# Gaius-Augustus/Augustus

Hardware: AMD Instinct MI355X
Metric: Mbp DNA decoded/sec (whole node), ab-initio human model (higher is better)
Workload: dtype f64; 1 GPU; synthetic uniform-random DNA, 100 contigs x 1000000 bp per GPU, --species=human ab initio (47 states, sample=0); pieces_in_flight_per_gpu=100, batches_in_flight_per_gpu=1

## Files before the change

augustus_amd/csrc/device/decoder.hip:

```cpp
#include <hip/hip_runtime.h>
#include <sys/mman.h>
#include <algorithm>
#include <map>
#include <array>
#include <cmath>
#include <unordered_map>
#include <cstdio>
#include <cstdlib>
#include <cstring>
#include <future>
#include <memory>
#include <mutex>
#include <set>
#include <string>
#include <system_error>
#include <thread>
#include <atomic>
#include <chrono>
#include <vector>
#include "kernels.h"
#include "dense.h"
#include "layout.h"
#include "launch.h"
#include "assmemo.h"
// ... 313 lines not shown

__global__ void __launch_bounds__(256) kTileCross(BatchView B) {
    const int64_t gt = (int64_t)blockIdx.x * 256 + threadIdx.x;
    if (gt < B.N / WAVE) tileCrossOne(B, gt);
}
__global__ void __launch_bounds__(64) kSegFinalize(BatchView B) {
    const int p = blockIdx.x * 64 + threadIdx.x;
    if (p < B.nPieces) segFinalizePiece(B, p);
}
__global__ void __launch_bounds__(64) kBacktrace(const DevTables *T, BatchView B) { backtracePiece(*T, B, blockIdx.x); }
struct GatherWin { int64_t o, gb0, poolOff, fxOff, fOff; int32_t b0, b1, g0, nSlots, nPl, r0, nRows, pad; };
__global__ void __launch_bounds__(256) kGatherWindows(BatchView V, const GatherWin *W, Item *outItems, uint64_t *outFx, const double *mat, double *outF, int S) {
    __shared__ uint32_t sc[256];
    __shared__ uint64_t running;
    const GatherWin w = W[blockIdx.x];
    const int t = threadIdx.x;
    if (t == 0) running = 0;
    __syncthreads();
    for (int base = w.b0; base <= w.b1; base += 256) {
        const int q = base + t;
        const uint32_t cnt = q <= w.b1 ? V.blkCnt[(w.gb0 + q) * 2 + 1] : 0;
        sc[t] = cnt;
        __syncthreads();
        for (int off = 1; off < 256; off <<= 1) {
            const uint32_t v = t >= off ? sc[t - off] : 0;
            __syncthreads();
            sc[t] += v;
            __syncthreads();
        }
        const uint64_t dst = (uint64_t)w.poolOff + running + (sc[t] - cnt);
        if (cnt) {
            const Item *src = V.items + V.blkOff[(w.gb0 + q) * 2 + 1];
            for (uint32_t i = 0; i < cnt; i++) outItems[dst + i] = src[i];
        }
        __syncthreads();
        if (t == 255) running += sc[255];
        __syncthreads();
    }
    const int64_t nFx = (int64_t)w.nPl * 2 * w.nSlots;
    for (int64_t i = t; i < nFx; i += 256) {
        const int pl = (int)(i / (2 * w.nSlots)), rev = (int)((i / w.nSlots) % 2), g = w.g0 + (int)(i % w.nSlots);
        outFx[w.fxOff + i] = V.fx[(int64_t)pl * V.N * NFX + fidx(w.o + g, rev ? FX_INR : FX_INF, NFX)];
    }
    if (mat && outF)
        for (int64_t i = t; i < (int64_t)w.nRows * S; i += 256) outF[w.fOff + i] = mat[(w.o + 1 + w.r0) * S + i];
}
__global__ void __launch_bounds__(256) kPatchItems(BatchView B, const uint64_t *idx, const double *te, int n) {
    const int i = blockIdx.x * blockDim.x + threadIdx.x;
    if (i < n) B.items[idx[i]].te = te[i];
}

namespace augx { namespace dev {
#define AUGX_BY_BLK(f, ...) do { if (blk == 8) f##8(__VA_ARGS__); else if (blk == 4) f##4(__VA_ARGS__); else f##2(__VA_ARGS__); } while (0)
void launchTrellis(int blk, int mode, bool ties, unsigned grid, hipStream_t st, const DevTables *T, const BatchView *B) { AUGX_BY_BLK(launchTrellis_, mode, ties, grid, st, T, B); }
void launchCand(int blk, bool multi, bool dense, unsigned grid, hipStream_t st, const DevTables *T, const BatchView &W) { AUGX_BY_BLK(launchCand_, multi, dense, grid, st, T, W); }
void launchForward(int blk, unsigned grid, hipStream_t st, const DevTables *T, const BatchView *B) { AUGX_BY_BLK(launchForward_, grid, st, T, B); }
void launchDense(int blk, int mode, bool ties, unsigned grid, hipStream_t st, const DevTables *T, const BatchView *B) { AUGX_BY_BLK(launchDense_, mode, ties, grid, st, T, B); }
void launchUtrDesc(int blk, unsigned grid, hipStream_t st, const DevTables *T, const BatchView &W) { AUGX_BY_BLK(launchUtrDesc_, grid, st, T, W); }
#undef AUGX_BY_BLK
}}

struct augx_decoder {
    const augx_model *model = nullptr;
    int device = 0;
    hipStream_t stream = nullptr;
    DevTables hostT;
    DevTables *dT = nullptr;
    std::vector<void *> tableBufs;
    bool debugCells = false;
    int blk = 8;
    int nCU = 256;
    int share = 1;
    std::multimap<size_t, void *> pool;
    std::unordered_map<void *, size_t> live;
    std::atomic<size_t> pooledBytes{0};
    std::mutex poolMu;
    std::vector<hipStream_t> copyStreams;
    bool dense = false;
    bool countNearTies = false;
    int64_t nearTies = 0, nearTiePieces = 0;
    double mallocSeconds = 0, mallocBytes = 0;
    bool exactMulti = true;
};

namespace {
int snippetCacheReplay(augx_decoder *d, augx_batch *b, int64_t &nPatched, bool fromLists, const double *mat);
int utrCachesReplay(augx_decoder *d, augx_batch *b, const double *mat, bool &rebuilt);
std::mutex g_regMu;
std::vector<augx_decoder *> g_decoders;
constexpr size_t POOL_CAP_BYTES = (size_t)250 << 30;
size_t sizeClass(size_t bytes) {
    if (bytes < ((size_t)1 << 20)) return (bytes + 4095) & ~(size_t)4095;
    size_t p2 = (size_t)1 << 20;
    while (p2 < bytes) p2 <<= 1;
    const size_t step = p2 >> 4;
    return (bytes + step - 1) / step * step;
}
void poolReleaseLocked(augx_decoder *d) {
    for (auto &kv : d->pool) (void)hipFree(kv.second);
    d->pool.clear();
    d->pooledBytes = 0;
}
void poolRelease(augx_decoder *d) {
    std::lock_guard<std::mutex> lk(d->poolMu);
    poolReleaseLocked(d);
}
hipError_t devMalloc(augx_decoder *d, void **out, size_t bytes) {
// ... 47 lines not shown
    d->pool.emplace(it->second, p);
    d->pooledBytes += it->second;
    d->live.erase(it);
}
struct DevBuf {
    augx_decoder *d = nullptr;
    void *p = nullptr;
    DevBuf() = default;
    DevBuf(DevBuf &&o) noexcept : d(o.d), p(o.p) { o.p = nullptr; }
    ~DevBuf() { reset(); }
    void reset() { devFree(d, p); p = nullptr; }
    explicit operator bool() const { return p != nullptr; }
    template <class T> T *as() const { return (T *)p; }
    int alloc(augx_decoder *dec, size_t bytes, const std::string &what) {
        reset();
        d = dec;
        const char *fail = getenv("AUGX_FAIL_ALLOC");
        const hipError_t e = fail && *fail && what.find(fail) != std::string::npos ? hipErrorOutOfMemory : devMalloc(d, &p, bytes);
        if (e == hipSuccess) return AUGX_OK;
        (void)hipGetLastError();
        p = nullptr;
        if (e == hipErrorOutOfMemory) { setLastError(what); return AUGX_E_NOMEM; }
        setLastError(std::string("HIP error: ") + hipGetErrorString(e) + " (" + what + ")");
        return AUGX_E_HIP;
    }
};
}


constexpr int NARR = 26;
struct augx_batch {
    augx_decoder *dec = nullptr;
    BatchLayout L;
    BatchView V;
    BatchView *dV = nullptr;
    std::vector<DevBuf> bufs;
    int32_t *blkMinMax = nullptr;
    int32_t *stairInfo = nullptr;
    int nPlAlloc = 0;
    int64_t listCapAlloc = 0;
    bool listsReady = false;
    int64_t *dListOffs = nullptr;
    DevBuf planeBufs[NARR];
    bool utrScanned = false;
    hipEvent_t ev[4] = {nullptr, nullptr, nullptr, nullptr};
    hipEvent_t evFwd = nullptr;
    uint64_t nItems = 0, nPairs = 0;
    DevBuf itemBuf;
    DevBuf udBuf;
    uint64_t nDescs = 0;
    bool decoded = false;
    bool itemsVerified = false;
    SegPlan plan;
    int chunkTotPlanes = 1;
    std::vector<int64_t> hListOffs;
    bool memoReplayed = false;
    DevBuf laSwBuf;
    size_t nLaSw = 0;
    std::vector<std::shared_ptr<augx::dev::AssMemoReplay>> memoOf;
};

namespace {

int ensureArrays(augx_batch *b, int nPl, int64_t listCap, bool *grown = nullptr) {
    if (nPl <= b->nPlAlloc && listCap <= b->listCapAlloc) return 0;
    if (grown) *grown = true;
    if (nPl < b->nPlAlloc) nPl = b->nPlAlloc;
    if (listCap < b->listCapAlloc) listCap = b->listCapAlloc;
    BatchView &V = b->V;
    const int64_t N = b->L.N, LC = listCap > 0 ? listCap : 1;
    struct Slot { void **field; size_t elem; int64_t count; int planes; };
    const Slot slots[NARR] = {
        {(void **)&V.fx, sizeof(uint64_t), N * NFX, nPl},          {(void **)&V.plsR, sizeof(double), N * 3, nPl},
        {(void **)&V.ldEnt, sizeof(IntronStart), LC, nPl},         {(void **)&V.rdEnt, sizeof(IntronStart), LC, nPl},
        {(void **)&V.laPls, sizeof(double), LC * 3, nPl},          {(void **)&V.laFx, sizeof(uint64_t), LC * 3, nPl},
        {(void **)&V.lrEt, sizeof(double), LC * 3, nPl},           {(void **)&V.lrFx, sizeof(uint64_t), LC * 3, nPl},
        {(void **)&V.atgD, sizeof(double), LC * 3, nPl},           {(void **)&V.atgFx, sizeof(uint64_t), LC, nPl},
        {(void **)&V.rsFx, sizeof(uint64_t), LC * 3, nPl},
        {(void **)&V.laPos, sizeof(int32_t), LC, 1},               {(void **)&V.laVal, sizeof(double), LC * 3, 1},
        {(void **)&V.lrPos, sizeof(int32_t), LC, 1},               {(void **)&V.lrVal, sizeof(double), LC * 3, 1},
        {(void **)&V.ldVal, sizeof(double), LC * 3, 1},            {(void **)&V.rdVal, sizeof(double), LC * 3, 1},
        {(void **)&V.atgPos, sizeof(int32_t), LC, 1},              {(void **)&V.rsPos, sizeof(int32_t), LC, 1},
        {(void **)&V.rsBegin, sizeof(double), LC, 1},
        {(void **)&V.tfSite, sizeof(USite), b->dec->dense ? LC : 1, 1}, {(void **)&V.laSite, sizeof(USite), b->dec->dense ? LC : 1, 1},
        {(void **)&V.fsSite, sizeof(USite), b->dec->dense ? LC : 1, 1}, {(void **)&V.lrSite, sizeof(USite), b->dec->dense ? LC : 1, 1},
        {(void **)&V.tmSite, sizeof(USite), b->dec->dense ? LC : 1, 1}, {(void **)&V.rtSite, sizeof(USite), b->dec->dense ? LC : 1, 1}};
    const std::string what = "augx: out of device memory for the candidate-list / per-GC-class arrays (" + std::to_string(nPl) + " classes in one piece); decode fewer bases per batch";
    for (int i = 0; i < NARR; i++) {
        const bool isN = i < 2;
        if (isN && nPl == b->nPlAlloc && b->planeBufs[i]) continue;
        if (const int rc = b->planeBufs[i].alloc(b->dec, (size_t)slots[i].planes * (size_t)slots[i].count * slots[i].elem, what)) {
            b->nPlAlloc = 0; b->listCapAlloc = 0;
            for (int k = 0; k < NARR; k++) { b->planeBufs[k].reset(); *slots[k].field = nullptr; }
            return rc;
        }
        *slots[i].field = b->planeBufs[i].p;
    }
    b->nPlAlloc = nPl;
    b->listCapAlloc = listCap;
    return 0;
}

}

extern "C" {

// ... 196 lines not shown
    if (!d->dense) {
        keep(V.bp, Z.N * SP);
        keep(V.bpChain, Z.N * 8);
    } else {
        keep(V.bpD, Z.N * d->hostT.S);
        keep(V.ufx, Z.N * NUFX); keep(V.ucnt, Z.N * NUCNT); keep(V.usig, Z.N * NUSIG);
    }
    if (d->debugCells || d->dense) keep(V.cells, Z.N * d->hostT.S);
    if (d->countNearTies) keep(V.nearTie, n);
    if (getenv("AUGX_PROF")) { keep(V.prof, (int64_t)n * 56 + 64); if (!rc && hipMemset(V.prof, 0, ((size_t)n * 56 + 64) * 8) != hipSuccess) { setLastError("augx_batch_create: hipMemset failed"); return AUGX_E_HIP; } }
    if (!d->dense) { keep(V.vig, Z.N); keep(V.longV, Z.N * 6); }
    keep(V.listCnt, n); keep(b->dListOffs, n + 1);
    V.listOffs = b->dListOffs;
    if (rc || (rc = ensureArrays(b.get(), 1, 0))) return rc;
    V.blk = d->blk;
    V.nBlk = Z.N / V.blk;
    keep(V.blkCnt, V.nBlk * 2); keep(V.blkSplit, V.nBlk * 3); keep(V.blkOff, V.nBlk * 2);
    keep(V.candAlloc, 1);
    if (d->dense && d->hostT.utr) { keep(V.udOff, V.nBlk); keep(V.udCnt, V.nBlk); }
    keep(V.lnv, n); keep(V.status, n); keep(V.finalState, n); keep(V.pathCount, n);
    {
        std::vector<double> v;
        {
            std::lock_guard<std::mutex> lk(g_tss0Mu);
            if (!g_tss0Of.empty() && d->dense && d->hostT.utr)
                for (int p = 0; p < n; p++) {
                    auto it = g_tss0Of.find(pieces[p].seq);
                    if (it == g_tss0Of.end()) continue;
                    if (v.empty()) v.assign((size_t)n * 2, std::nan(""));
                    v[(size_t)p * 2] = it->second[0]; v[(size_t)p * 2 + 1] = it->second[1];
                }
        }
        if (!v.empty()) {
            double *dv = nullptr;
            keep(dv, (int64_t)n * 2);
            if (rc) return rc;
            if (hipMemcpy(dv, v.data(), sizeof(double) * v.size(), hipMemcpyHostToDevice) != hipSuccess) { setLastError("augx_batch_create: upload failed"); return AUGX_E_HIP; }
            V.tss0 = dv;
        }
    }
    keep(V.pathRec, Z.pathCap * 3);
    b->plan = planSegments(L, d->model->m.t, d->nCU / d->share > 0 ? d->nCU / d->share : 1, d->dense ? -1 : 0);
    SegDesc *dSegs = nullptr; int32_t *dSeg0 = nullptr;
    const int nSegs = (int)b->plan.segs.size();
    keep(dSegs, nSegs); keep(dSeg0, n + 1);
    V.nSegs = nSegs; V.segs = dSegs; V.pieceSeg0 = dSeg0; V.segCheckTiles = b->plan.checkTiles;
    if (const char *e = getenv("AUGX_SEG_CHECK_TILES")) V.segCheckTiles = atoi(e);
    keep(V.segStop, nSegs); keep(V.segStatus, nSegs); keep(V.segD, nSegs); keep(V.brkPos, nSegs); keep(V.brkOff, nSegs);
    keep(V.segStop2, nSegs); keep(V.segD2, nSegs); keep(V.pieceCovered, n);
    if (b->plan.cut()) {
        keep(V.ckRing, (int64_t)nSegs * 2 * WAVE * SP); keep(V.ckCol, Z.N / WAVE * SP);
        keep(V.tileMinEop, Z.N / WAVE); keep(V.tileCross, Z.N / WAVE);
    }
    keep(b->dV, 1);
    if (rc) return rc;
    const double tAlloc = getenv("AUGX_TIMING") ? std::chrono::duration<double>(std::chrono::steady_clock::now().time_since_epoch()).count() : 0.0;
    HIP_TRY(hipMemcpy(dOff, L.off.data(), sizeof(int64_t) * (n + 1), hipMemcpyHostToDevice));
    HIP_TRY(hipMemcpy(dLen, L.len.data(), sizeof(int32_t) * n, hipMemcpyHostToDevice));
    HIP_TRY(hipMemcpy(dIk, L.initKind.data(), sizeof(int32_t) * n, hipMemcpyHostToDevice));
    HIP_TRY(hipMemcpy(dTk, L.termKind.data(), sizeof(int32_t) * n, hipMemcpyHostToDevice));
    HIP_TRY(hipMemcpy(dCp, L.chunkPiece.data(), sizeof(int32_t) * L.nChunks, hipMemcpyHostToDevice));
    HIP_TRY(hipMemcpy(dSegs, b->plan.segs.data(), sizeof(SegDesc) * nSegs, hipMemcpyHostToDevice));
    HIP_TRY(hipMemcpy(dSeg0, b->plan.pieceSeg0.data(), sizeof(int32_t) * (n + 1), hipMemcpyHostToDevice));
    HIP_TRY(hipMemset(dRaw, 'n', (size_t)Z.N));
    HIP_TRY(hipMemset(V.gcPlane, 0, (size_t)Z.N));
    for (int p = 0; p < n; p++)
        HIP_TRY(hipMemcpy(dRaw + L.off[p] + 1, pieces[p].seq, (size_t)L.len[p], hipMemcpyHostToDevice));
    HIP_TRY(hipMemcpy(b->dV, &V, sizeof(BatchView), hipMemcpyHostToDevice));
    for (auto &e : b->ev) HIP_TRY(hipEventCreate(&e));
    if (tAlloc > 0) fprintf(stderr, "augx timing:       batch created: uploads + events %.3f s after the allocations (hipMalloc calls of this decoder so far: %.3f s for %.1f GB)\n",
                            std::chrono::duration<double>(std::chrono::steady_clock::now().time_since_epoch()).count() - tAlloc, d->mallocSeconds, d->mallocBytes / 1e9);
    *out = b.release();
    return AUGX_OK;
}

int augx_batch_decode(augx_decoder *d, augx_batch *b) {
    if (!d || !b) { setLastError("augx_batch_decode: NULL argument"); return AUGX_E_ARG; }
    HIP_TRY(hipSetDevice(d->device));
    const BatchView &V = b->V;
    const int n = V.nPieces;
    const unsigned gridN = (unsigned)((V.N + 255) / 256);
    hipStream_t st = d->stream;
    HIP_TRY(hipEventRecord(b->ev[0], st));
    b->memoReplayed = false;
    b->memoOf.clear();
    hipLaunchKernelGGL(kEncode, dim3(gridN), dim3(256), 0, st, V);
    int rc;
    const bool timingFirst = !b->decoded && getenv("AUGX_TIMING") != nullptr;
    auto nowS = [] { return std::chrono::duration<double>(std::chrono::steady_clock::now().time_since_epoch()).count(); };
    double tf[6] = {0, 0, 0, 0, 0, 0};
    if (timingFirst) tf[0] = nowS();
    const unsigned nScan = (unsigned)(V.N / SCAN_T);
    hipLaunchKernelGGL(kSiteScanTotals, dim3(nScan), dim3(SCAN_T), 0, st, d->dT, V, V.chunkTot);
    hipLaunchKernelGGL(kChunkOffsets, dim3(n, 1, NSF), dim3(64), 0, st, V.chunkTot, V, NSF, NCNT);
    hipLaunchKernelGGL(kSiteScanApply, dim3(nScan), dim3(SCAN_T), 0, st, d->dT, V, V.chunkTot);
    if (!b->listsReady) hipLaunchKernelGGL(kListCount, dim3((n + 63) / 64), dim3(64), 0, st, V);
    b->utrScanned = false;
    auto utrScan = [&]() {
        hipLaunchKernelGGL(kUtrScanTotals, dim3(nScan), dim3(SCAN_T), 0, st, d->dT, V, V.chunkTot);
        hipLaunchKernelGGL(kChunkOffsets, dim3(n, 1, NUF), dim3(64), 0, st, V.chunkTot, V, NUF, NUF);
        hipLaunchKernelGGL(kUtrScanApply, dim3(nScan), dim3(SCAN_T), 0, st, d->dT, V, V.chunkTot);
        b->utrScanned = true;
    };
    if (!b->decoded) {
    hipLaunchKernelGGL(kWindowClass, dim3(gridN), dim3(256), 0, st, d->dT, V, b->blkMinMax);
    hipLaunchKernelGGL(kClassFinal, dim3(n), dim3(64), 0, st, V, b->blkMinMax);
    HIP_TRY(hipGetLastError());
    {
        BatchView &W = b->V;
        HIP_TRY(hipMemsetAsync(b->stairInfo, 0, 2 * sizeof(int32_t), st));
        hipLaunchKernelGGL(kStairs, dim3(n), dim3(256), 0, st, d->dT, V, b->stairInfo);
        int32_t info[2] = {0, 0};
        HIP_TRY(hipMemcpyAsync(info, b->stairInfo, sizeof info, hipMemcpyDeviceToHost, st));
        HIP_TRY(hipStreamSynchronize(st));
        int nPl = info[0] > 1 ? info[0] : 1;
        if (timingFirst) tf[1] = nowS();
// ... 83 lines not shown
            if ((rc = b->udBuf.alloc(d, (size_t)W.udCap * sizeof(UDesc), "augx_batch_decode: out of device memory for the UTR descriptors; decode fewer bases per batch"))) return rc;
            W.ud = b->udBuf.as<UDesc>();
            HIP_TRY(hipMemcpyAsync(b->dV, &W, sizeof(BatchView), hipMemcpyHostToDevice, st));
        }
        const bool steady = b->decoded && b->itemBuf && b->nItems > 0 && (uint64_t)W.itemCap >= b->nItems && b->itemsVerified;
        for (int attempt = 0;; attempt++) {
            HIP_TRY(hipMemsetAsync(W.candAlloc, 0, sizeof(CandAlloc), st));
            const bool multi = W.nPl > 1;
            if (utrDesc) {
                const unsigned nGrp = (unsigned)(W.N / (NT / 16));
                launchUtrDesc(d->blk, nGrp, st, d->dT, W);
            }
            launchCand(d->blk, multi, d->dense, nWg, st, d->dT, W);
            HIP_TRY(hipGetLastError());
            if (steady) break;
            CandAlloc tot;
            HIP_TRY(hipMemcpyAsync(&tot, W.candAlloc, sizeof tot, hipMemcpyDeviceToHost, st));
            HIP_TRY(hipStreamSynchronize(st));
            b->nPairs = tot.pairs; b->nItems = tot.items; b->nDescs = tot.descs;
            const bool itemsFit = (int64_t)tot.items <= W.itemCap, descsFit = !utrDesc || (int64_t)tot.descs <= W.udCap;
            if (itemsFit && descsFit) { b->itemsVerified = true; break; }
            if (attempt > 0) { setLastError("augx_batch_decode: candidate buffers overflowed twice"); return AUGX_E_HIP; }
            if (!itemsFit) {
                W.itemCap = (int64_t)tot.items + 64;
                if ((rc = b->itemBuf.alloc(d, (size_t)W.itemCap * sizeof(Item), "augx_batch_decode: out of device memory for the candidate buffer (" + std::to_string(tot.items) + " candidates); decode fewer bases per batch"))) return rc;
                W.items = b->itemBuf.as<Item>();
            }
            if (!descsFit) {
                W.udCap = (int64_t)tot.descs + 64;
                if ((rc = b->udBuf.alloc(d, (size_t)W.udCap * sizeof(UDesc), "augx_batch_decode: out of device memory for the UTR descriptors; decode fewer bases per batch"))) return rc;
                W.ud = b->udBuf.as<UDesc>();
            }
            HIP_TRY(hipMemcpyAsync(b->dV, &W, sizeof(BatchView), hipMemcpyHostToDevice, st));
        }
    }
    if (timingFirst) {
        tf[4] = nowS();
        fprintf(stderr, "augx timing:       first decode of the batch, host side: class kernels + stairs %.3f s, stairs on the host + list sizes %.3f s, per-class / list arrays (%d planes) %.3f s, "
                        "prep launches + candidate buffer + candidates counted %.3f s (hipMalloc so far: %.3f s for %.1f GB)\n", tf[1] - tf[0], tf[2] - tf[1], b->V.nPl, tf[3] - tf[2], tf[4] - tf[3],
                d->mallocSeconds, d->mallocBytes / 1e9);
    }
    if (b->plan.cut()) hipLaunchKernelGGL(kTileCross, dim3((unsigned)((V.N / WAVE + 255) / 256)), dim3(256), 0, st, V);
    HIP_TRY(hipEventRecord(b->ev[1], st));
    auto runTrellis = [&]() -> int {
    if (d->dense) {
        launchDense(d->blk, 0, V.nearTie, (unsigned)n, st, d->dT, b->dV);
        HIP_TRY(hipGetLastError());
        HIP_TRY(hipEventRecord(b->ev[2], st));
        hipLaunchKernelGGL(kDenseBacktrace, dim3(n), dim3(64), 0, st, d->dT, V);
        HIP_TRY(hipGetLastError());
        return AUGX_OK;
    }
    HIP_TRY(hipMemsetAsync(V.segStatus, 0, sizeof(int32_t) * V.nSegs, st));
#define AUGX_LAUNCH_TRELLIS(MODE_, grid_) launchTrellis(d->blk, MODE_, V.nearTie, (unsigned)(grid_), st, d->dT, b->dV)
    AUGX_LAUNCH_TRELLIS(0, V.nSegs);
    if (b->plan.cut()) {
        HIP_TRY(hipMemsetAsync(V.segStop2, 0xFF, sizeof(int32_t) * V.nSegs, st));
        HIP_TRY(hipMemsetAsync(V.pieceCovered, 0xFF, sizeof(int32_t) * n, st));
        AUGX_LAUNCH_TRELLIS(1, V.nSegs);
        for (int round = 0; round < SEG_CONT_ROUNDS; round++) AUGX_LAUNCH_TRELLIS(2, n);
        AUGX_LAUNCH_TRELLIS(3, n);
    }
#undef AUGX_LAUNCH_TRELLIS
    hipLaunchKernelGGL(kSegFinalize, dim3((n + 63) / 64), dim3(64), 0, st, V);
    HIP_TRY(hipGetLastError());
    HIP_TRY(hipEventRecord(b->ev[2], st));
    hipLaunchKernelGGL(kBacktrace, dim3(n), dim3(64), 0, st, d->dT, V);
    HIP_TRY(hipGetLastError());
    return AUGX_OK;
    };
    int rcT = runTrellis();
    if (rcT) return rcT;
    b->decoded = true;
    if (d->exactMulti && b->nPlAlloc > 1) {
        int64_t nPatched = 0;
        int rc2;
        const bool timing = getenv("AUGX_TIMING") != nullptr;
        auto now = [] { return std::chrono::duration<double>(std::chrono::steady_clock::now().time_since_epoch()).count(); };
        if (timing) (void)hipStreamSynchronize(st);
        const double t0 = timing ? now() : 0.0;
        bool sitesRebuilt = false;
        try {
            rc2 = d->dense ? snippetCacheReplay(d, b, nPatched, false, b->V.cells) : snippetCacheReplay(d, b, nPatched, true, nullptr);
            if (!rc2 && d->dense && d->hostT.utr) rc2 = utrCachesReplay(d, b, b->V.cells, sitesRebuilt);
        } catch (const std::exception &e) { setLastError(std::string("augx_batch_decode: replay of the reference's caches: ") + e.what()); return AUGX_E_NOMEM; }
        if (rc2) return rc2;
        const double t1 = timing ? now() : 0.0;
        if ((nPatched > 0 || sitesRebuilt) && (rc2 = runTrellis())) return rc2;
        if (timing) {
            (void)hipStreamSynchronize(st);
            fprintf(stderr, "augx timing:     pieces with several GC classes: snippet-cache replay %.3f s (%lld candidate terms rebuilt), second trellis run %.3f s\n", t1 - t0, (long long)nPatched, now() - t1);
        }
    }
    HIP_TRY(hipEventRecord(b->ev[3], st));
    return AUGX_OK;
}

int augx_batch_sync(augx_decoder *d) {
    if (!d) return AUGX_E_ARG;
    HIP_TRY(hipSetDevice(d->device));
    HIP_TRY(hipStreamSynchronize(d->stream));
    return AUGX_OK;
}

int augx_batch_kernel_ms(augx_decoder *d, augx_batch *b, float *prep_ms, float *trellis_ms, float *back_ms) {
    if (!d || !b || !b->decoded) return AUGX_E_ARG;
    HIP_TRY(hipSetDevice(d->device));
    HIP_TRY(hipEventSynchronize(b->ev[3]));
    float a = 0, c = 0, e = 0;
    HIP_TRY(hipEventElapsedTime(&a, b->ev[0], b->ev[1]));
    HIP_TRY(hipEventElapsedTime(&c, b->ev[1], b->ev[2]));
    HIP_TRY(hipEventElapsedTime(&e, b->ev[2], b->ev[3]));
    if (prep_ms) *prep_ms = a;
    if (trellis_ms) *trellis_ms = c;
    if (back_ms) *back_ms = e;
    if (b->V.prof && d->dense) {
        std::vector<uint64_t> h((size_t)b->L.nPieces * 56 + 64);
        HIP_TRY(hipMemcpy(h.data(), b->V.prof, h.size() * 8, hipMemcpyDeviceToHost));
        fprintf(stderr, "kDense Mcycles/piece:");
        for (int i = 0; i < 11; i++) {
            double sum = 0;
            for (int p = 0; p < b->L.nPieces; p++) sum += (double)h[(size_t)p * 56 + i];
            fprintf(stderr, " [%d]=%.2f", i, sum / b->L.nPieces / 1e6);
        }
        fprintf(stderr, "  (wavefront 1: 0 loop, 1 stage 1: fixed-lag states + staging, 2 ... wait for the UTR units, 3 stage 2: records + early chains' inputs, 4 forward sums, "
                        "5 stage 3: cells + early chain runs, 6 last-base redo, 7 stage 4: late chains, 8 RTERMINAL records, 9 their cells, 10 fence)\n");
    } else if (b->V.prof) {
        std::vector<uint64_t> h((size_t)b->L.nPieces * 56 + 64);
        HIP_TRY(hipMemcpy(h.data(), b->V.prof, h.size() * 8, hipMemcpyDeviceToHost));
        static const char *role[5] = {"work0", "work1", "work2", "chain", "far"};
        for (int w = 0; w < 5; w++) {
            fprintf(stderr, "trellis %-6s Mcycles/piece:", role[w]);
            for (int i = 0; i < 8; i++) {
                double sum = 0;
                for (int p = 0; p < b->L.nPieces; p++) sum += (double)h[((size_t)p * 5 + w) * 8 + i];
                fprintf(stderr, " [%d]=%.2f", i, sum / b->L.nPieces / 1e6);
            }
            fprintf(stderr, "  (0 tile wait, 1 flag wait, 2 role work, 3 chain, 4 item load, 5 scan, 6 publish, 7 item setup)\n");
        }
        {
            const uint64_t *cp = &h[(size_t)b->L.nPieces * 56];
            const double nw = (double)(cp[4] ? cp[4] : 1);
            fprintf(stderr, "kCand cycles per wavefront (= tile; avg over %.0f): %.0f  (describe + count %.0f, reserve %.0f)\n", nw, cp[0] / nw, cp[1] / nw, cp[2] / nw);
        }
        {
            const uint64_t *ts = &h[(size_t)b->L.nPieces * 40];
            fprintf(stderr, "block 1000 of piece 0 (cycles): F %lld..%lld  I1 %lld..%lld  I2 %lld..%lld  late %lld..%lld  chain %lld..%lld\n",
                    0LL, (long long)(ts[1] - ts[0]), (long long)(ts[2] - ts[0]), (long long)(ts[3] - ts[0]), (long long)(ts[4] - ts[0]),
                    (long long)(ts[5] - ts[0]), (long long)(ts[6] - ts[0]), (long long)(ts[7] - ts[0]), (long long)(ts[8] - ts[0]), (long long)(ts[9] - ts[0]));
            fprintf(stderr, "end of tile 124 (cycles after worker 0 left its last block): igenic tail %lld..%lld  worker-0 tail done %lld  far tail done %lld  barrier passed %lld  (block 1000: late starts %lld)\n",
                    (long long)(ts[11] - ts[10]), (long long)(ts[12] - ts[10]), (long long)(ts[13] - ts[10]), (long long)(ts[14] - ts[10]), (long long)(ts[15] - ts[10]), (long long)(ts[6] - ts[10]));
        }
    }
    return AUGX_OK;
}

int augx_batch_paths(augx_decoder *d, augx_batch *b, augx_path *out) {
    if (!d || !b || !out || !b->decoded) { setLastError("augx_batch_paths: bad argument"); return AUGX_E_ARG; }
    HIP_TRY(hipSetDevice(d->device));
    HIP_TRY(hipStreamSynchronize(d->stream));
    const BatchView &V = b->V;
    const int n = V.nPieces;
    std::vector<double> lnv(n);
    std::vector<int32_t> status(n), count(n);
    HIP_TRY(hipMemcpy(lnv.data(), V.lnv, sizeof(double) * n, hipMemcpyDeviceToHost));
// ... 812 lines not shown
```

augustus_amd/csrc/device/k_trellis.hip:

```cpp
#include "kernels.h"
#include "launch.h"

using namespace augx;
using namespace augx::dev;

template <int BLK, int MODE, bool TIES> __global__ void __launch_bounds__(NT) kTrellis(const DevTables *__restrict__ T, const BatchView *__restrict__ B) {
    __shared__ TrellisLds lds;
    if constexpr (!TIES) {
        const int w = __builtin_amdgcn_readfirstlane((int)(threadIdx.x >> 6));
        switch (w) {
            case 0: trellisPiece<BLK, MODE, TIES, 0>(*T, *B, lds, blockIdx.x); break;
            case 1: trellisPiece<BLK, MODE, TIES, 1>(*T, *B, lds, blockIdx.x); break;
            case 2: trellisPiece<BLK, MODE, TIES, 2>(*T, *B, lds, blockIdx.x); break;
            case 3: trellisPiece<BLK, MODE, TIES, 3>(*T, *B, lds, blockIdx.x); break;
            case 4: trellisPiece<BLK, MODE, TIES, 4>(*T, *B, lds, blockIdx.x); break;
            case 5: trellisPiece<BLK, MODE, TIES, 5>(*T, *B, lds, blockIdx.x); break;
            case 6: trellisPiece<BLK, MODE, TIES, 6>(*T, *B, lds, blockIdx.x); break;
            default: trellisPiece<BLK, MODE, TIES, 7>(*T, *B, lds, blockIdx.x); break;
        }
    } else
        trellisPiece<BLK, MODE, TIES>(*T, *B, lds, blockIdx.x);
}

namespace augx { namespace dev {
void AUGX_TU_NAME(launchTrellis_)(int mode, bool ties, unsigned grid, hipStream_t st, const DevTables *T, const BatchView *B) {
    constexpr int BLK = AUGX_TU_BLK;
#define L(MODE_) do { if (ties) hipLaunchKernelGGL((kTrellis<BLK, MODE_, true>), dim3(grid), dim3(NT), 0, st, T, B); \
                      else hipLaunchKernelGGL((kTrellis<BLK, MODE_, false>), dim3(grid), dim3(NT), 0, st, T, B); } while (0)
    switch (mode) { case 0: L(0); break; case 1: L(1); break; case 2: L(2); break; default: L(3); break; }
#undef L
}
}}
```

augustus_amd/csrc/device/launch.h:

```cpp
#pragma once
#include <hip/hip_runtime.h>
#include "dp.h"

namespace augx { namespace dev {
void launchTrellis(int blk, int mode, bool ties, unsigned grid, hipStream_t st, const DevTables *T, const BatchView *B);
void launchCand(int blk, bool multi, bool dense, unsigned grid, hipStream_t st, const DevTables *T, const BatchView &W);
void launchForward(int blk, unsigned grid, hipStream_t st, const DevTables *T, const BatchView *B);
void launchDense(int blk, int mode, bool ties, unsigned grid, hipStream_t st, const DevTables *T, const BatchView *B);
void launchUtrDesc(int blk, unsigned grid, hipStream_t st, const DevTables *T, const BatchView &W);

#define AUGX_DECL_TU(BLK_)                                                                                                     \
    void launchTrellis_##BLK_(int mode, bool ties, unsigned grid, hipStream_t st, const DevTables *T, const BatchView *B);     \
    void launchCand_##BLK_(bool multi, bool dense, unsigned grid, hipStream_t st, const DevTables *T, const BatchView &W);     \
    void launchForward_##BLK_(unsigned grid, hipStream_t st, const DevTables *T, const BatchView *B);                          \
    void launchDense_##BLK_(int mode, bool ties, unsigned grid, hipStream_t st, const DevTables *T, const BatchView *B);       \
    void launchUtrDesc_##BLK_(unsigned grid, hipStream_t st, const DevTables *T, const BatchView &W);
AUGX_DECL_TU(8) AUGX_DECL_TU(4) AUGX_DECL_TU(2)
#undef AUGX_DECL_TU
#define AUGX_TU_CAT2(a, b) a##b
#define AUGX_TU_CAT(a, b) AUGX_TU_CAT2(a, b)
#define AUGX_TU_NAME(f) AUGX_TU_CAT(f, AUGX_TU_BLK)
}}
```

augustus_amd/csrc/device/layout.h:

```cpp
#pragma once
#include <cstdlib>
#include <cstring>
#include <stdexcept>
#include <string>
#include <vector>
#include "dp.h"

namespace augx {
namespace dev {

struct BatchLayout {
    int nPieces = 0;
    int64_t N = 0;
    int nChunks = 0;
    std::vector<int64_t> off;
    std::vector<int32_t> len, initKind, termKind, chunkPiece;
    void build(const augx_piece *pieces, int n) {
        nPieces = n;
        off.assign(n + 1, 0);
        len.resize(n); initKind.resize(n); termKind.resize(n);
        for (int p = 0; p < n; p++) {
            if (pieces[p].len < 1 || pieces[p].len >= 2900000) throw std::runtime_error("augx: piece length out of range (device pieces are shorter than 2.9 Mbp; lower --maxDNAPieceSize)");
            len[p] = (int32_t)pieces[p].len;
            initKind[p] = pieces[p].init_kind;
            termKind[p] = pieces[p].term_kind;
            int64_t slots = (int64_t)len[p] + 1 + 8;
            slots = (slots + CHUNK - 1) / CHUNK * CHUNK;
            off[p + 1] = off[p] + slots;
        }
        N = off[n];
        nChunks = (int)(N / CHUNK);
        chunkPiece.resize(nChunks);
        for (int p = 0; p < n; p++)
            for (int64_t ch = off[p] / CHUNK; ch < off[p + 1] / CHUNK; ch++) chunkPiece[ch] = p;
    }
};

constexpr int STAIR_RUNS = 4096;
constexpr int SCAN_T = 256;

inline int stairsPlanes(const uint8_t *wc, int n, int win, std::vector<uint8_t> &plane, int32_t planeCls[MAXPL]) {
    if (win > n || win < 1) win = n;
    const int half = win / 2, last = n - win;
    std::vector<int> st, cl;
    for (int s0 = 0; s0 <= last;) {
        const uint8_t c = wc[s0];
        int s1 = s0 + 1;
        const uint64_t pat = 0x0101010101010101ull * c;
        while (s1 + 8 <= last + 1) {
            uint64_t w;
            memcpy(&w, wc + s1, 8);
            if (w != pat) break;
            s1 += 8;
        }
        while (s1 <= last && wc[s1] == c) s1++;
        st.push_back(s0 == 0 ? 0 : s0 + half);
        cl.push_back(c);
        s0 = s1;
    }
    const int R = (int)st.size();
    for (int k = 2; k < R; k++)
        if (st[k] - st[k - 1] < 1000 && st[k - 1] > 0 && cl[k - 2] == cl[k]) cl[k - 1] = cl[k];
    int nPl = 0, map[256];
    for (int i = 0; i < 256; i++) map[i] = -1;
    plane.resize((size_t)n);
    for (int k = 0; k < R; k++) {
        int &m = map[cl[k]];
        if (m < 0) {
            if (nPl >= MAXPL) return -1;
            planeCls[nPl] = cl[k];
            m = nPl++;
        }
        const int e = k + 1 < R ? st[k + 1] : n;
        memset(plane.data() + st[k], m, (size_t)(e - st[k]));
    }
    return nPl;
}

inline int64_t listOffsets(const int32_t *listCnt, int nPieces, std::vector<int64_t> &offs) {
    offs.assign((size_t)nPieces + 1, 0);
    for (int p = 0; p < nPieces; p++) offs[p + 1] = offs[p] + (((int64_t)listCnt[p] + 1 + 63) / 64) * 64;
    return offs[nPieces] + 64;
}

constexpr int SEG_CONT_ROUNDS = 3;
struct SegPlan {
    std::vector<SegDesc> segs;
    std::vector<int32_t> pieceSeg0;
    int checkTiles = 0;
    bool cut() const { return segs.size() + 1 > pieceSeg0.size(); }
};
inline int segCheckTiles(const augx_tables &t) {
    int reach = t.max_exon_len > t.d ? t.max_exon_len : t.d;
    reach += t.W + t.U + 64;
    return (reach + WAVE - 1) / WAVE + 4;
}
inline bool segmentsSupported(const augx_tables &t) {
    const int dL = t.d - 2 - t.De - t.As - 2 - t.U;
    return t.state_kind[t.synch_state] == AUGX_K_IGENIC && dL >= 4 * WAVE && t.reachable[t.synch_state];
}
inline SegPlan planSegments(const BatchLayout &L, const augx_tables &t, int slots, int segTiles = 0) {
    SegPlan P;
    P.checkTiles = segCheckTiles(t);
    const int n = L.nPieces;
    if (const char *e = getenv("AUGX_SEG_LEN")) { const long v = atol(e); segTiles = v <= 0 ? -1 : (int)((v + WAVE - 1) / WAVE); }
    const int minSeg = 5 * P.checkTiles;
    std::vector<int> tiles(n);
    int64_t total = 0;
    int maxTiles = 0;
    for (int p = 0; p < n; p++) { tiles[p] = (L.len[p] + WAVE - 1) / WAVE; total += tiles[p]; if (tiles[p] > maxTiles) maxTiles = tiles[p]; }
    if (!segmentsSupported(t)) segTiles = -1;
    auto countFor = [&](int st, int p) {
        int k = (tiles[p] + st / 2) / st;
        while (k > 1 && tiles[p] / k < minSeg) k--;
        return k < 1 ? 1 : k;
    };
    if (segTiles == 0) {
        const int64_t fixLen = 450;
        int64_t bestCost = -1;
        int best = -1;
        for (int k = 1; k <= 64; k++) {
            int st = (maxTiles + k - 1) / k;
            if (k > 1 && st < minSeg) break;
            int64_t nSeg = 0, nFix = 0, longest = 0;
            for (int p = 0; p < n; p++) {
                const int kp = k == 1 ? 1 : countFor(st, p);
                nSeg += kp; nFix += kp - 1;
                const int64_t len = (tiles[p] + kp - 1) / kp;
                if (len > longest) longest = len;
            }
            int64_t cost = (nSeg + slots - 1) / slots * longest + (nFix + slots - 1) / slots * fixLen;
            if (k > 1) cost += cost / 6;
            if (bestCost < 0 || cost < bestCost) { bestCost = cost; best = k == 1 ? -1 : st; }
        }
        segTiles = best;
    }
    if (segTiles > 0 && segTiles < minSeg) segTiles = minSeg;
    std::vector<int> kOf(n, 1);
    if (segTiles > 0) {
        int64_t nSeg = 0;
        for (int p = 0; p < n; p++) { kOf[p] = countFor(segTiles, p); nSeg += kOf[p]; }
        int extra = nSeg > slots ? (int)((slots - nSeg % slots) % slots) : 0;
        if (extra > 0 && extra <= n / 4 + 1)
            for (int p = 0; p < n && extra > 0; p++)
                if (kOf[p] > 1 && tiles[p] / (kOf[p] + 1) >= minSeg) { kOf[p]++; extra--; }
    }
    P.pieceSeg0.assign((size_t)n + 1, 0);
    for (int p = 0; p < n; p++) {
        const int kp = kOf[p];
        P.pieceSeg0[p] = (int32_t)P.segs.size();
        for (int k = 0; k < kp; k++) {
            SegDesc d;
            d.piece = p; d.k = k;
            d.t0 = (int32_t)((int64_t)tiles[p] * k / kp);
            d.t1 = (int32_t)((int64_t)tiles[p] * (k + 1) / kp);
            d.tlim = d.t1 - P.checkTiles - 2;
            d.pad = 0;
            P.segs.push_back(d);
        }
    }
    P.pieceSeg0[n] = (int32_t)P.segs.size();
    return P;
}

struct BatchSizes {
    int64_t N, nChunks, nPieces, pathCap;
    explicit BatchSizes(const BatchLayout &L) {
        N = L.N; nChunks = L.nChunks; nPieces = L.nPieces;
        pathCap = N / 8 + 64 * (int64_t)L.nPieces + 64;
    }
};

inline long long forwardCellCandidates(const augx_tables &t) {
    int len = t.max_exon_len > t.d ? t.max_exon_len : t.d;
    if (t.utr_max_exon_len > len) len = t.utr_max_exon_len;
    if (t.utr_max3single > len) len = t.utr_max3single;
    if (t.utr_max3term > len) len = t.utr_max3term;
    return (long long)AUGX_MAX_ANC * ((long long)len + 1);
}
static_assert((long long)AUGX_MAX_ANC * (0x3FFF + 1) <= FWD_SUM_TERMS, "the lengths 14-bit back pointers admit fit the forward sum");
inline void checkForwardSum(const augx_tables &t) {
    if (forwardCellCandidates(t) > FWD_SUM_TERMS) throw std::runtime_error("augx: exon or intron lengths too large for the fixed-point sums of the forward pass");
}

inline void checkModelSupported(const augx_tables &t, int BLK) {
    checkForwardSum(t);
    if (t.S > SP) throw std::runtime_error("augx: model has more than 48 states: not for the wavefront layout of the trellis kernel (models with UTR states or two intergenic states go to the dense kernels, modelIsDense below)");
    int dL = t.d - 2 - t.De - t.As - 2 - t.U;
    if (dL >= LONG_RING || dL <= BLK || (dL > WAVE - BLK && dL < WAVE)) throw std::runtime_error("augx: intron d out of the supported range");
    if (t.Ds + 2 + t.De < BLK || t.As + 2 + t.Ae + t.U < BLK) throw std::runtime_error("augx: splice-site windows shorter than a trellis block");
    if (t.As + 2 + t.Ae + t.U > 63 || t.Ds + 2 + t.De > 63) throw std::runtime_error("augx: splice-site windows too long");
    if (t.max_exon_len + t.W + 64 > 0x3FFF) throw std::runtime_error("augx: maxexonlength too large for 14-bit back pointers");
    if (t.d > 0x3FFF) throw std::runtime_error("augx: intron d too large");
    int nFixed = 0, nVar = 0, nChain = 0;
    for (int s = 0; s < t.S; s++) {
        int kind = t.state_kind[s];
        if (t.reachable[s]) {
            bool fixedLag = kind == AUGX_K_LONGDSS || kind == AUGX_K_RLONGDSS || kind == AUGX_K_LONGASS || kind == AUGX_K_RLONGASS ||
                            kind == AUGX_K_EQUALD || kind == AUGX_K_REQUALD;
            bool chain = kind == AUGX_K_IGENIC || kind == AUGX_K_GEOMETRIC || kind == AUGX_K_RGEOMETRIC;
            if (fixedLag) { nFixed++; if (t.n_anc[s] > 2) throw std::runtime_error("augx: fixed-length intron state with more than 2 ancestors"); }
            else if (chain) { nChain++; if (t.n_anc[s] > 5) throw std::runtime_error("augx: single-base state with more than 5 ancestors"); }
            else nVar++;
        }
        bool var3 = kind == AUGX_K_INTERNAL || kind == AUGX_K_TERMINAL || kind == AUGX_K_RINTERNAL || kind == AUGX_K_RINITIAL;
        if (var3 && t.n_anc[s] > 3) throw std::runtime_error("augx: exon state with more than 3 ancestors");
        if (var3)
            for (int a = 0; a < t.n_anc[s]; a++)
                for (int b2 = 0; b2 < a; b2++)
                    if (t.state_win[t.anc[s][a]] == t.state_win[t.anc[s][b2]])
                        throw std::runtime_error("augx: exon state with two ancestors of the same reading frame");
        if ((kind == AUGX_K_LESSD || kind == AUGX_K_RLESSD || kind == AUGX_K_SINGLE || kind == AUGX_K_INITIAL ||
             kind == AUGX_K_RSINGLE || kind == AUGX_K_RTERMINAL) && t.n_anc[s] != 1)
// ... 201 lines not shown
```

Before: 489.5 Mbp/s.

## Plan trellis segments by simulated makespan and launch longest segments first

Measured after the change: 407.1 Mbp/s. -16.8%, worse.

```diff
diff --git a/augustus_amd/csrc/device/decoder.hip b/augustus_amd/csrc/device/decoder.hip
--- a/augustus_amd/csrc/device/decoder.hip
+++ b/augustus_amd/csrc/device/decoder.hip
@@ -389,7 +389,7 @@
 
 namespace augx { namespace dev {
 #define AUGX_BY_BLK(f, ...) do { if (blk == 8) f##8(__VA_ARGS__); else if (blk == 4) f##4(__VA_ARGS__); else f##2(__VA_ARGS__); } while (0)
-void launchTrellis(int blk, int mode, bool ties, unsigned grid, hipStream_t st, const DevTables *T, const BatchView *B) { AUGX_BY_BLK(launchTrellis_, mode, ties, grid, st, T, B); }
+void launchTrellis(int blk, int mode, bool ties, unsigned grid, hipStream_t st, const DevTables *T, const BatchView *B, const int32_t *order) { AUGX_BY_BLK(launchTrellis_, mode, ties, grid, st, T, B, order); }
 void launchCand(int blk, bool multi, bool dense, unsigned grid, hipStream_t st, const DevTables *T, const BatchView &W) { AUGX_BY_BLK(launchCand_, multi, dense, grid, st, T, W); }
 void launchForward(int blk, unsigned grid, hipStream_t st, const DevTables *T, const BatchView *B) { AUGX_BY_BLK(launchForward_, grid, st, T, B); }
 void launchDense(int blk, int mode, bool ties, unsigned grid, hipStream_t st, const DevTables *T, const BatchView *B) { AUGX_BY_BLK(launchDense_, mode, ties, grid, st, T, B); }
@@ -543,6 +543,7 @@
     bool decoded = false;
     bool itemsVerified = false;
     SegPlan plan;
+    int32_t *dSegOrder = nullptr;
     int chunkTotPlanes = 1;
     std::vector<int64_t> hListOffs;
     bool memoReplayed = false;
@@ -845,6 +846,8 @@
         keep(V.ckRing, (int64_t)nSegs * 2 * WAVE * SP); keep(V.ckCol, Z.N / WAVE * SP);
         keep(V.tileMinEop, Z.N / WAVE); keep(V.tileCross, Z.N / WAVE);
     }
+    std::vector<int32_t> segOrder;
+    if (b->plan.cut()) { segOrder = segLaunchOrder(b->plan.segs); keep(b->dSegOrder, nSegs); }
     keep(b->dV, 1);
     if (rc) return rc;
     const double tAlloc = getenv("AUGX_TIMING") ? std::chrono::duration<double>(std::chrono::steady_clock::now().time_since_epoch()).count() : 0.0;
@@ -855,6 +858,7 @@
     HIP_TRY(hipMemcpy(dCp, L.chunkPiece.data(), sizeof(int32_t) * L.nChunks, hipMemcpyHostToDevice));
     HIP_TRY(hipMemcpy(dSegs, b->plan.segs.data(), sizeof(SegDesc) * nSegs, hipMemcpyHostToDevice));
     HIP_TRY(hipMemcpy(dSeg0, b->plan.pieceSeg0.data(), sizeof(int32_t) * (n + 1), hipMemcpyHostToDevice));
+    if (b->dSegOrder) HIP_TRY(hipMemcpy(b->dSegOrder, segOrder.data(), sizeof(int32_t) * nSegs, hipMemcpyHostToDevice));
     HIP_TRY(hipMemset(dRaw, 'n', (size_t)Z.N));
     HIP_TRY(hipMemset(V.gcPlane, 0, (size_t)Z.N));
     for (int p = 0; p < n; p++)
@@ -1044,7 +1048,7 @@
         return AUGX_OK;
     }
     HIP_TRY(hipMemsetAsync(V.segStatus, 0, sizeof(int32_t) * V.nSegs, st));
-#define AUGX_LAUNCH_TRELLIS(MODE_, grid_) launchTrellis(d->blk, MODE_, V.nearTie, (unsigned)(grid_), st, d->dT, b->dV)
+#define AUGX_LAUNCH_TRELLIS(MODE_, grid_) launchTrellis(d->blk, MODE_, V.nearTie, (unsigned)(grid_), st, d->dT, b->dV, (MODE_) == 0 ? b->dSegOrder : nullptr)
     AUGX_LAUNCH_TRELLIS(0, V.nSegs);
     if (b->plan.cut()) {
         HIP_TRY(hipMemsetAsync(V.segStop2, 0xFF, sizeof(int32_t) * V.nSegs, st));
@@ -1103,6 +1107,20 @@
     HIP_TRY(hipEventElapsedTime(&a, b->ev[0], b->ev[1]));
     HIP_TRY(hipEventElapsedTime(&c, b->ev[1], b->ev[2]));
     HIP_TRY(hipEventElapsedTime(&e, b->ev[2], b->ev[3]));
+    if (getenv("AUGX_TIMING") && b->plan.cut()) {
+        std::vector<int32_t> stop(b->plan.segs.size());
+        HIP_TRY(hipMemcpy(stop.data(), b->V.segStop, sizeof(int32_t) * stop.size(), hipMemcpyDeviceToHost));
+        long long nFix = 0, sum = 0, longest = 0, gaveUp = 0;
+        for (size_t s = 0; s < stop.size(); s++) {
+            const SegDesc &sd = b->plan.segs[s];
+            if (sd.k == 0) continue;
+            const long long last = stop[s] <= -2 ? -2 - (long long)stop[s] : stop[s], len = last - sd.t0 + 1;
+            nFix++; sum += len; gaveUp += stop[s] <= -2;
+            if (len > longest) longest = len;
+        }
+        fprintf(stderr, "augx timing:       fix-ups: %zu segments for %d pieces, %lld fix-ups of %.0f tiles on average, the longest %lld tiles, %lld gave up\n",
+                stop.size(), b->L.nPieces, nFix, nFix ? (double)sum / nFix : 0.0, longest, gaveUp);
+    }
     if (prep_ms) *prep_ms = a;
     if (trellis_ms) *trellis_ms = c;
     if (back_ms) *back_ms = e;
diff --git a/augustus_amd/csrc/device/k_trellis.hip b/augustus_amd/csrc/device/k_trellis.hip
--- a/augustus_amd/csrc/device/k_trellis.hip
+++ b/augustus_amd/csrc/device/k_trellis.hip
@@ -4,29 +4,30 @@
 using namespace augx;
 using namespace augx::dev;
 
-template <int BLK, int MODE, bool TIES> __global__ void __launch_bounds__(NT) kTrellis(const DevTables *__restrict__ T, const BatchView *__restrict__ B) {
+template <int BLK, int MODE, bool TIES> __global__ void __launch_bounds__(NT) kTrellis(const DevTables *__restrict__ T, const BatchView *__restrict__ B, const int32_t *__restrict__ order) {
     __shared__ TrellisLds lds;
+    const int sg = order ? order[blockIdx.x] : (int)blockIdx.x;
     if constexpr (!TIES) {
         const int w = __builtin_amdgcn_readfirstlane((int)(threadIdx.x >> 6));
         switch (w) {
-            case 0: trellisPiece<BLK, MODE, TIES, 0>(*T, *B, lds, blockIdx.x); break;
-            case 1: trellisPiece<BLK, MODE, TIES, 1>(*T, *B, lds, blockIdx.x); break;
-            case 2: trellisPiece<BLK, MODE, TIES, 2>(*T, *B, lds, blockIdx.x); break;
-            case 3: trellisPiece<BLK, MODE, TIES, 3>(*T, *B, lds, blockIdx.x); break;
-            case 4: trellisPiece<BLK, MODE, TIES, 4>(*T, *B, lds, blockIdx.x); break;
-            case 5: trellisPiece<BLK, MODE, TIES, 5>(*T, *B, lds, blockIdx.x); break;
-            case 6: trellisPiece<BLK, MODE, TIES, 6>(*T, *B, lds, blockIdx.x); break;
-            default: trellisPiece<BLK, MODE, TIES, 7>(*T, *B, lds, blockIdx.x); break;
+            case 0: trellisPiece<BLK, MODE, TIES, 0>(*T, *B, lds, sg); break;
+            case 1: trellisPiece<BLK, MODE, TIES, 1>(*T, *B, lds, sg); break;
+            case 2: trellisPiece<BLK, MODE, TIES, 2>(*T, *B, lds, sg); break;
+            case 3: trellisPiece<BLK, MODE, TIES, 3>(*T, *B, lds, sg); break;
+            case 4: trellisPiece<BLK, MODE, TIES, 4>(*T, *B, lds, sg); break;
+            case 5: trellisPiece<BLK, MODE, TIES, 5>(*T, *B, lds, sg); break;
+            case 6: trellisPiece<BLK, MODE, TIES, 6>(*T, *B, lds, sg); break;
+            default: trellisPiece<BLK, MODE, TIES, 7>(*T, *B, lds, sg); break;
         }
     } else
-        trellisPiece<BLK, MODE, TIES>(*T, *B, lds, blockIdx.x);
+        trellisPiece<BLK, MODE, TIES>(*T, *B, lds, sg);
 }
 
 namespace augx { namespace dev {
-void AUGX_TU_NAME(launchTrellis_)(int mode, bool ties, unsigned grid, hipStream_t st, const DevTables *T, const BatchView *B) {
+void AUGX_TU_NAME(launchTrellis_)(int mode, bool ties, unsigned grid, hipStream_t st, const DevTables *T, const BatchView *B, const int32_t *order) {
     constexpr int BLK = AUGX_TU_BLK;
-#define L(MODE_) do { if (ties) hipLaunchKernelGGL((kTrellis<BLK, MODE_, true>), dim3(grid), dim3(NT), 0, st, T, B); \
-                      else hipLaunchKernelGGL((kTrellis<BLK, MODE_, false>), dim3(grid), dim3(NT), 0, st, T, B); } while (0)
+#define L(MODE_) do { if (ties) hipLaunchKernelGGL((kTrellis<BLK, MODE_, true>), dim3(grid), dim3(NT), 0, st, T, B, order); \
+                      else hipLaunchKernelGGL((kTrellis<BLK, MODE_, false>), dim3(grid), dim3(NT), 0, st, T, B, order); } while (0)
     switch (mode) { case 0: L(0); break; case 1: L(1); break; case 2: L(2); break; default: L(3); break; }
 #undef L
 }
diff --git a/augustus_amd/csrc/device/launch.h b/augustus_amd/csrc/device/launch.h
--- a/augustus_amd/csrc/device/launch.h
+++ b/augustus_amd/csrc/device/launch.h
@@ -3,14 +3,14 @@
 #include "dp.h"
 
 namespace augx { namespace dev {
-void launchTrellis(int blk, int mode, bool ties, unsigned grid, hipStream_t st, const DevTables *T, const BatchView *B);
+void launchTrellis(int blk, int mode, bool ties, unsigned grid, hipStream_t st, const DevTables *T, const BatchView *B, const int32_t *order = nullptr);
 void launchCand(int blk, bool multi, bool dense, unsigned grid, hipStream_t st, const DevTables *T, const BatchView &W);
 void launchForward(int blk, unsigned grid, hipStream_t st, const DevTables *T, const BatchView *B);
 void launchDense(int blk, int mode, bool ties, unsigned grid, hipStream_t st, const DevTables *T, const BatchView *B);
 void launchUtrDesc(int blk, unsigned grid, hipStream_t st, const DevTables *T, const BatchView &W);
 
 #define AUGX_DECL_TU(BLK_)                                                                                                     \
-    void launchTrellis_##BLK_(int mode, bool ties, unsigned grid, hipStream_t st, const DevTables *T, const BatchView *B);     \
+    void launchTrellis_##BLK_(int mode, bool ties, unsigned grid, hipStream_t st, const DevTables *T, const BatchView *B, const int32_t *order); \
     void launchCand_##BLK_(bool multi, bool dense, unsigned grid, hipStream_t st, const DevTables *T, const BatchView &W);     \
     void launchForward_##BLK_(unsigned grid, hipStream_t st, const DevTables *T, const BatchView *B);                          \
     void launchDense_##BLK_(int mode, bool ties, unsigned grid, hipStream_t st, const DevTables *T, const BatchView *B);       \
diff --git a/augustus_amd/csrc/device/layout.h b/augustus_amd/csrc/device/layout.h
--- a/augustus_amd/csrc/device/layout.h
+++ b/augustus_amd/csrc/device/layout.h
@@ -1,6 +1,9 @@
 #pragma once
+#include <algorithm>
 #include <cstdlib>
 #include <cstring>
+#include <functional>
+#include <queue>
 #include <stdexcept>
 #include <string>
 #include <vector>
@@ -99,11 +102,42 @@
     const int dL = t.d - 2 - t.De - t.As - 2 - t.U;
     return t.state_kind[t.synch_state] == AUGX_K_IGENIC && dL >= 4 * WAVE && t.reachable[t.synch_state];
 }
+inline std::vector<int32_t> segLaunchOrder(const std::vector<SegDesc> &segs) {
+    std::vector<int32_t> order(segs.size());
+    for (size_t i = 0; i < order.size(); i++) order[i] = (int32_t)i;
+    std::stable_sort(order.begin(), order.end(), [&](int32_t a, int32_t b) { return segs[a].t1 - segs[a].t0 > segs[b].t1 - segs[b].t0; });
+    return order;
+}
+constexpr int64_t SEG_FIX_TILES = 900;
+inline int64_t segPass1Makespan(const std::vector<SegDesc> &segs, int slots) {
+    if (slots < 1) slots = 1;
+    const std::vector<int32_t> order = segLaunchOrder(segs);
+    if ((size_t)slots >= segs.size()) return segs.empty() ? 0 : segs[order[0]].t1 - segs[order[0]].t0;
+    std::priority_queue<int64_t, std::vector<int64_t>, std::greater<int64_t>> freeAt;
+    for (int i = 0; i < slots; i++) freeAt.push(0);
+    int64_t end = 0;
+    for (int32_t sg : order) {
+        const int64_t t = freeAt.top() + (segs[sg].t1 - segs[sg].t0);
+        freeAt.pop(); freeAt.push(t);
+        if (t > end) end = t;
+    }
+    return end;
+}
+inline int64_t segPlanCost(const std::vector<SegDesc> &segs, int nPieces, int slots) {
+    if (slots < 1) slots = 1;
+    const int64_t nFix = (int64_t)segs.size() - nPieces;
+    int64_t cost = segPass1Makespan(segs, slots) + (nFix + slots - 1) / slots * SEG_FIX_TILES;
+    if (nFix > 0) cost += cost / 6;
+    return cost;
+}
+
 inline SegPlan planSegments(const BatchLayout &L, const augx_tables &t, int slots, int segTiles = 0) {
     SegPlan P;
     P.checkTiles = segCheckTiles(t);
     const int n = L.nPieces;
     if (const char *e = getenv("AUGX_SEG_LEN")) { const long v = atol(e); segTiles = v <= 0 ? -1 : (int)((v + WAVE - 1) / WAVE); }
+    if (const char *e = getenv("AUGX_SEG_SLOTS")) { const int v = atoi(e); if (v > 0) slots = v; }
+    if (slots < 1) slots = 1;
     const int minSeg = 5 * P.checkTiles;
     std::vector<int> tiles(n);
     int64_t total = 0;
@@ -115,50 +149,68 @@
         while (k > 1 && tiles[p] / k < minSeg) k--;
         return k < 1 ? 1 : k;
     };
-    if (segTiles == 0) {
-        const int64_t fixLen = 450;
+    auto addSeg = [&](std::vector<SegDesc> &v, int p, int k, int t0, int t1) {
+        SegDesc d;
+        d.piece = p; d.k = k; d.t0 = t0; d.t1 = t1; d.tlim = t1 - P.checkTiles - 2; d.pad = 0;
+        v.push_back(d);
+    };
+    auto uniform = [&](int st, bool whole) {
+        std::vector<int> kOf(n, 1);
+        if (st > 0) {
+            int64_t nSeg = 0;
+            for (int p = 0; p < n; p++) { kOf[p] = countFor(st, p); nSeg += kOf[p]; }
+            int extra = whole && nSeg > slots ? (int)((slots - nSeg % slots) % slots) : 0;
+            if (extra > 0 && extra <= n / 4 + 1)
+                for (int p = 0; p < n && extra > 0; p++)
+                    if (kOf[p] > 1 && tiles[p] / (kOf[p] + 1) >= minSeg) { kOf[p]++; extra--; }
+        }
+        std::vector<SegDesc> v;
+        for (int p = 0; p < n; p++)
+            for (int k = 0; k < kOf[p]; k++) addSeg(v, p, k, (int32_t)((int64_t)tiles[p] * k / kOf[p]), (int32_t)((int64_t)tiles[p] * (k + 1) / kOf[p]));
+        return v;
+    };
+    auto packed = [&](int64_t load) {
+        std::vector<SegDesc> v;
+        if (load < minSeg) load = minSeg;
+        int64_t room = load;
+        for (int p = 0; p < n; p++) {
+            int pos = 0, k = 0;
+            while (pos < tiles[p]) {
+                const int64_t rest = tiles[p] - pos;
+                if (rest > room && room < minSeg) { room = load; continue; }
+                if (rest <= room || rest - room < minSeg) {
+                    addSeg(v, p, k, pos, tiles[p]);
+                    room -= rest;
+                    break;
+                }
+                addSeg(v, p, k++, pos, pos + (int)room);
+                pos += (int)room;
+                room = load;
+            }
+            if (room <= 0) room = load;
+        }
+        return v;
+    };
+    if (segTiles != 0) P.segs = uniform(segTiles > 0 && segTiles < minSeg ? minSeg : segTiles, true);
+    else if (maxTiles < 2 * minSeg) P.segs = uniform(-1, false);
+    else {
         int64_t bestCost = -1;
-        int best = -1;
-        for (int k = 1; k <= 64; k++) {
-            int st = (maxTiles + k - 1) / k;
-            if (k > 1 && st < minSeg) break;
-            int64_t nSeg = 0, nFix = 0, longest = 0;
-            for (int p = 0; p < n; p++) {
-                const int kp = k == 1 ? 1 : countFor(st, p);
-                nSeg += kp; nFix += kp - 1;
-                const int64_t len = (tiles[p] + kp - 1) / kp;
-                if (len > longest) longest = len;
-            }
-            int64_t cost = (nSeg + slots - 1) / slots * longest + (nFix + slots - 1) / slots * fixLen;
-            if (k > 1) cost += cost / 6;
-            if (bestCost < 0 || cost < bestCost) { bestCost = cost; best = k == 1 ? -1 : st; }
-        }
-        segTiles = best;
-    }
-    if (segTiles > 0 && segTiles < minSeg) segTiles = minSeg;
-    std::vector<int> kOf(n, 1);
-    if (segTiles > 0) {
-        int64_t nSeg = 0;
-        for (int p = 0; p < n; p++) { kOf[p] = countFor(segTiles, p); nSeg += kOf[p]; }
-        int extra = nSeg > slots ? (int)((slots - nSeg % slots) % slots) : 0;
-        if (extra > 0 && extra <= n / 4 + 1)
-            for (int p = 0; p < n && extra > 0; p++)
-                if (kOf[p] > 1 && tiles[p] / (kOf[p] + 1) >= minSeg) { kOf[p]++; extra--; }
+        auto offer = [&](std::vector<SegDesc> &&v) {
+            const int64_t cost = segPlanCost(v, n, slots);
+            if (bestCost < 0 || cost < bestCost || (cost == bestCost && v.size() < P.segs.size())) { bestCost = cost; P.segs = std::move(v); }
+        };
+        offer(uniform(-1, false));
+        for (int k = 2; k <= 64; k++) {
+            const int st = (maxTiles + k - 1) / k;
+            if (st < minSeg) break;
+            offer(uniform(st, false));
+            offer(uniform(st, true));
+        }
+        int64_t mMax = total / minSeg < slots ? total / minSeg : slots;
+        for (int64_t m = mMax; m >= 1 && m >= mMax - mMax / 4; m--) offer(packed((total + m - 1) / m));
     }
     P.pieceSeg0.assign((size_t)n + 1, 0);
-    for (int p = 0; p < n; p++) {
-        const int kp = kOf[p];
-        P.pieceSeg0[p] = (int32_t)P.segs.size();
-        for (int k = 0; k < kp; k++) {
-            SegDesc d;
-            d.piece = p; d.k = k;
-            d.t0 = (int32_t)((int64_t)tiles[p] * k / kp);
-            d.t1 = (int32_t)((int64_t)tiles[p] * (k + 1) / kp);
-            d.tlim = d.t1 - P.checkTiles - 2;
-            d.pad = 0;
-            P.segs.push_back(d);
-        }
-    }
+    for (size_t s = P.segs.size(); s-- > 0;) P.pieceSeg0[P.segs[s].piece] = (int32_t)s;
     P.pieceSeg0[n] = (int32_t)P.segs.size();
     return P;
 }
```
